# Samleo8/RadarSLAMPy

Measured on AMD Instinct MI355X. Metric: radar scan-pairs/sec (400x3768 polar), higher is better.
Workload: dtype u8/f32/f64

## Files before the change

profiles/time_doh.py:

```python
#!/usr/bin/env python3
import os, sys
sys.path.insert(0, os.path.dirname(os.path.dirname(os.path.abspath(__file__))))
import numpy as np
from radarslampy_amd import _ffi, synth
if os.environ.get("ROAM_LIB"):
    _ffi.LIB_PATH = os.path.abspath(os.environ["ROAM_LIB"])
from radarslampy_amd.engine import Engine
B = int(sys.argv[1]) if len(sys.argv) > 1 else 512
recs, poses, feat = synth.make_sequence(5, 2, n_static=460, n_movers=24, distortion=True)
ctx = _ffi.Context(0)
eng = Engine(B, 2 * B, ctx=ctx, retrack_on_device=True, retrack_slots=B)
for t in range(2):
    eng.upload_scan(t, recs[t])
for b in range(1, B):
    for t in range(2):
        eng.copy_scan(b * 2 + t, t)
eng.synchronize()
for b in range(B):
    eng.init_lane(b, b * 2, feat[:40], poses[0])
eng.step(np.arange(B, dtype=np.int32) * 2 + 1)
eng.synchronize()
for k in os.environ.get("KERNELS", "doh_integral,doh_det_maxima").split(","):
    ms, by = eng.time_kernel(k, 3)
    print(f"{k}: {ms:.2f} ms per {B} detections = {ms*1e3/B:.1f} us each, {by/ms/1e6:.0f} GB/s algorithmic")
eng.close(); ctx.close()
```

radarslampy_amd/csrc/retrack_det.hip:

```cpp
#include "doh_common.h"
#include "retrack_geom.h"

__device__ __forceinline__ void rt_push_maxima(const RtArgs &a, int ls, int r, int c, uint32_t bits, double v0, double v1)
{
#pragma unroll
    for (int l = 0; l < 2; l++)
        if ((bits >> l) & 1u) {
            const int o = atomicAdd(&a.cand_n[ls], 1);
            if (o < BP_MAX_PTS) {
                a.cand_rc[(int64_t)ls * BP_MAX_PTS + o] = ((uint32_t)r << 16) | ((uint32_t)c << 2) | (uint32_t)(l + 1);
                a.cand_val[(int64_t)ls * BP_MAX_PTS + o] = l ? v1 : v0;
            }
        }
}

#define SD_RING 64
#define SD_DUP 8
#define SD_PITCHB (SD_BP * 8)
#define SD_SPLIT 36
#define SD_THREADS (512 * SD_HALVES)
#define SD_RING_BYTES ((SD_RING + SD_DUP) * SD_PITCHB)
#define SD_M2_ROWS (SD_T + 2)
#define SD_LDS_BYTES (SD_RING_BYTES + 2 * SD_M2_ROWS * SD_PC * 8)
#define SD_NST ((SD_T * SD_BP + SD_THREADS - 1) / SD_THREADS)
extern __shared__ __align__(16) char sd_smem[];

#define SD_SCALE 0.0009765625
#define SD_UNSCALE 1024.0
__device__ __forceinline__ double sd_box(double a, double d, double b, double c)
{
    const double t = __dsub_rn(__dadd_rn(a, d), b);
    double r;
    asm("v_add_f64 %0, %1, -%2 clamp" : "=v"(r) : "v"(t), "v"(c));
    return r;
}
__device__ __forceinline__ double sd_max(double x, double y)
{
    double r;
    asm("v_max_f64 %0, %1, %2" : "=v"(r) : "v"(x), "v"(y));
    return r;
}
template <int SIZE> __device__ __forceinline__ double sd_wi() { return __dmul_rn(__ddiv_rn(__ddiv_rn(1.0, (double)SIZE), (double)SIZE), SD_UNSCALE); }

__device__ __forceinline__ double sd_ldr(const uint32_t (&ca)[12], const uint32_t (&cb)[12], int row, int j)
{
    const int rr = ((row % SD_RING) + SD_RING) % SD_RING;
    return rr < SD_SPLIT ? *reinterpret_cast<const double *>(sd_smem + (ca[j] + rr * SD_PITCHB))
                         : *reinterpret_cast<const double *>(sd_smem + (cb[j] + (rr - SD_SPLIT) * SD_PITCHB));
}

template <int PH>
__device__ __forceinline__ void sd_tile_fast(const uint32_t (&ca)[12], const uint32_t (&cb)[12], double (&d0)[SD_T / 8], double (&d1)[SD_T / 8])
{
    static_assert(SD_T == 16, "two positions per thread and step");
    double v[2][2][4];
    auto issue = [&](int i, double(&o)[2][4]) {
        const int L = (i >> 2) & 1, q = i & 3;
        const int SIZE = L ? 30 : 15, s2 = (SIZE - 1) / 2, s3 = SIZE / 3;
        const int ra = q < 2 ? -s3 + 1 : (q == 2 ? -s2 : -(s3 / 2)), rb = ra + (q < 2 ? 2 * s3 - 1 : (q == 2 ? SIZE : s3));
        const int ja = 6 * L + (q == 0 ? 0 : (q == 1 ? 2 : 4)), jb = ja + 1;
#pragma unroll
        for (int k = 0; k < 2; k++) {
            const int R0 = SD_T * PH + 8 * k;
            o[k][0] = sd_ldr(ca, cb, R0 + ra, ja); o[k][1] = sd_ldr(ca, cb, R0 + rb, jb);
            o[k][2] = sd_ldr(ca, cb, R0 + ra, jb); o[k][3] = sd_ldr(ca, cb, R0 + rb, ja);
        }
    };
    issue(0, v[0]);
    double mid[2] = {0.0, 0.0}, dxx[2] = {0.0, 0.0};
#pragma unroll
    for (int i = 0; i < 8; i++) {
        if (i + 1 < 8) issue(i + 1, v[(i + 1) & 1]);
        const int L = (i >> 2) & 1, q = i & 3;
        const double(&x)[2][4] = v[i & 1];
        double t0 = __dadd_rn(x[0][0], x[0][1]), t1 = __dadd_rn(x[1][0], x[1][1]);
        t0 = __dsub_rn(t0, x[0][2]); t1 = __dsub_rn(t1, x[1][2]);
        double b0, b1;
        asm("v_add_f64 %0, %1, -%2 clamp" : "=v"(b0) : "v"(t0), "v"(x[0][3]));
        asm("v_add_f64 %0, %1, -%2 clamp" : "=v"(b1) : "v"(t1), "v"(x[1][3]));
        if (q == 0 || q == 2) { mid[0] = b0; mid[1] = b1; }
        else {
            const double w_i = L ? sd_wi<30>() : sd_wi<15>();
            double m0 = __dmul_rn(3.0, b0), m1 = __dmul_rn(3.0, b1);
            double e0 = __dsub_rn(mid[0], m0), e1 = __dsub_rn(mid[1], m1);
            e0 = __dmul_rn(-e0, w_i); e1 = __dmul_rn(-e1, w_i);
            if (q == 1) { dxx[0] = e0; dxx[1] = e1; }
            else if (L) { d1[0] = __dmul_rn(dxx[0], e0); d1[1] = __dmul_rn(dxx[1], e1); }
            else { d0[0] = __dmul_rn(dxx[0], e0); d0[1] = __dmul_rn(dxx[1], e1); }
        }
        __builtin_amdgcn_sched_barrier(0);
    }
}

template <int SIZE, int L>
__device__ __forceinline__ double sd_det_rows(const uint32_t (&ca)[12], int w8, int r, int H)
{
    constexpr int s2 = (SIZE - 1) / 2, s3 = SIZE / 3, w = SIZE, J = 6 * L;
    const double w_i = sd_wi<SIZE>();
    auto ld = [&](int row, int j) { return *reinterpret_cast<const double *>(sd_smem + (ca[j] + (uint32_t)(((row & (SD_RING - 1)) - w8) * SD_PITCHB))); };
    const int xa = clipi(r - s3 + 1, 0, H - 1), xb = clipi(xa + 2 * s3 - 1, 0, H - 1);
    double mid = sd_box(ld(xa, J + 0), ld(xb, J + 1), ld(xa, J + 1), ld(xb, J + 0));
    double side = sd_box(ld(xa, J + 2), ld(xb, J + 3), ld(xa, J + 3), ld(xb, J + 2));
    double dxx = __dsub_rn(mid, __dmul_rn(3.0, side));
    dxx = __dmul_rn(-dxx, w_i);
    const int ya = clipi(r - s2, 0, H - 1), yb = clipi(ya + w, 0, H - 1), za = clipi(r - s3 / 2, 0, H - 1), zb = clipi(za + s3, 0, H - 1);
    mid = sd_box(ld(ya, J + 4), ld(yb, J + 5), ld(ya, J + 5), ld(yb, J + 4));
    side = sd_box(ld(za, J + 4), ld(zb, J + 5), ld(za, J + 5), ld(zb, J + 4));
    double dyy = __dsub_rn(mid, __dmul_rn(3.0, side));
    dyy = __dmul_rn(-dyy, w_i);
    return __dmul_rn(dxx, dyy);
}

template <int SIZE>
__device__ __forceinline__ double sd_dxy(double det, int r, int c, int H, int W, int cbase)
{
    constexpr int s3 = SIZE / 3;
    const double w_i = sd_wi<SIZE>();
    const int r0 = clipi(r - s3, 0, H - 1), r1 = clipi(r0 + s3, 0, H - 1), r2 = clipi(r + 1, 0, H - 1), r3 = clipi(r2 + s3, 0, H - 1);
    const int c0 = clipi(c - s3, 0, W - 1), c1 = clipi(c0 + s3, 0, W - 1), c2 = clipi(c + 1, 0, W - 1), c3 = clipi(c2 + s3, 0, W - 1);
    auto at = [&](int rr, int cc) { return *reinterpret_cast<const double *>(sd_smem + (((rr & (SD_RING - 1)) * SD_BP + (cc - cbase)) * 8)); };
    const double tl = sd_box(at(r0, c0), at(r1, c1), at(r0, c1), at(r1, c0));
    const double br = sd_box(at(r2, c2), at(r3, c3), at(r2, c3), at(r3, c2));
    const double bl = sd_box(at(r0, c2), at(r1, c3), at(r0, c3), at(r1, c2));
    const double tr = sd_box(at(r2, c0), at(r3, c1), at(r2, c1), at(r3, c0));
    double dxy = __dsub_rn(__dsub_rn(__dadd_rn(bl, tr), tl), br);
    dxy = __dmul_rn(-dxy, w_i);
    return __dsub_rn(det, __dmul_rn(0.81, __dmul_rn(dxy, dxy)));
}

__global__ __launch_bounds__(256) void rt_darktab_kernel(const uint32_t *__restrict__ map, int W, int cols, uint32_t *__restrict__ tab)
{
    const int H = W, strip = blockIdx.x, t = blockIdx.y, c0 = strip * SD_OUT;
    const int ra = max(SD_T * t - SD_HL, 0), rb = min(SD_T * t + SD_T - 1 + SD_HR, H - 1);
    const int xa = max(c0 - 1 - SD_HL, 0), xb = min(c0 - 1 + SD_PC - 1 + SD_HR, W - 1);
    const int nx = xb - xa + 1, n = max(0, rb - ra + 1) * max(0, nx);
    int lit = 0;
    for (int i = threadIdx.x; i < n; i += 256) {
        const int r = ra + i / nx, c = xa + i % nx;
        if ((int)(map[(int64_t)r * W + c] & 4095u) < cols) lit = 1;
    }
    lit = __syncthreads_or(lit);
    if (threadIdx.x == 0 && !lit) atomicOr(&tab[strip * SD_DT_WORDS + (t >> 5)], 1u << (t & 31));
}
__global__ __launch_bounds__(256) void rt_darkskip_kernel(int nt, uint32_t *__restrict__ tab)
{
    uint32_t *T = tab + blockIdx.x * SD_DT_WORDS;
    const int t = threadIdx.x;
    auto dark = [&](int q) { return q < 0 || q >= nt || ((T[q >> 5] >> (q & 31)) & 1u); };
    auto skip = [&](int j) { return dark(j - 1) && dark(j) && dark(j + 1); };
    if (skip(t + 4)) atomicOr(&T[8 + (t >> 5)], 1u << (t & 31));
    if (t == 0) {
        int first = nt, last = -1;
        for (int q = 0; q < nt; q++)
            if (!dark(q)) { if (first == nt) first = q; last = q; }
        T[16] = (uint32_t)first; T[17] = (uint32_t)last;
    }
}

template <int P> struct SdTag { static constexpr int value = P; };

__global__ __launch_bounds__(SD_THREADS) void rt_det_strip_kernel(RtArgs a, int first, int P, int nstrips)
{
    const int nact = min(P, max(0, *a.rt_n - first));
    if (a.fused && rt_one_sweep(a, first)) return;
    const int total = nact * nstrips, per = (total + 7) >> 3;
    const int xcd = blockIdx.x & 7, jq = blockIdx.x >> 3;
    const int work = xcd * per + jq;
    if (jq >= per || work >= total) return;
    const int ls = work / nstrips, strip = work - ls * nstrips;
    const int W = a.W, H = a.W, SP = a.SP;
    const double thr = a.threshold;
    typedef const uint32_t __attribute__((address_space(4))) *SdConstPtr;
    const SdConstPtr dtab = (SdConstPtr)(uintptr_t)(a.darktab + strip * SD_DT_WORDS);
    uint32_t dk_w = 0, skf_w = 0;
    const double *__restrict__ S = a.S + (int64_t)ls * SP * W;
    const int tid = threadIdx.x, lane = tid & 63;
    const int wave = __builtin_amdgcn_readfirstlane(tid >> 6), w8 = wave & 7, half = wave >> 3;
    const int c0 = strip * SD_OUT, cbase = c0 - 1 - SD_HL;
    const int pc = half * 64 + lane, c = c0 - 1 + pc;
    const bool cvalid = c >= 0 && c < W;
    const bool wave_live = c0 - 1 + half * 64 < W;
    constexpr int M2ROW = SD_PC * 8, M2BUF = SD_M2_ROWS * M2ROW;
    const uint32_t mb = (uint32_t)(SD_RING_BYTES + w8 * M2ROW + pc * 8);
    auto m2at = [&](int buf, int row, int dc) -> double & { return *reinterpret_cast<double *>(sd_smem + (mb + (uint32_t)(buf * M2BUF + (row - w8) * M2ROW + dc * 8))); };
    uint32_t ca[12], cb[12];
    {
        constexpr int off[6][2] = {{-7, 15}, {-2, 5}, {-4, 9}, {-14, 30}, {-5, 10}, {-9, 19}};
#pragma unroll
        for (int q = 0; q < 6; q++) {
            const int x0 = clipi(c + off[q][0], 0, W - 1), x1 = clipi(x0 + off[q][1], 0, W - 1);
            ca[2 * q] = (uint32_t)((w8 * SD_BP + (x0 - cbase)) * 8);
            ca[2 * q + 1] = (uint32_t)((w8 * SD_BP + (x1 - cbase)) * 8);
        }
#pragma unroll
        for (int q = 0; q < 12; q++) cb[q] = ca[q] + SD_SPLIT * SD_PITCHB;
    }
    const bool strip_inside = cbase >= 0 && cbase + SD_BP <= W;
    uint32_t goff[SD_NST], loff[SD_NST];
    int srow[SD_NST], scol[SD_NST];
#pragma unroll
    for (int j = 0; j < SD_NST; j++) {
        const int e = tid + SD_THREADS * j;
        srow[j] = e / SD_BP; scol[j] = e - srow[j] * SD_BP;
        goff[j] = (uint32_t)((srow[j] * SP + scol[j]) * 8);
        loff[j] = (uint32_t)(srow[j] * SD_PITCHB + scol[j] * 8);
    }
    double stage[2][SD_NST];
    const int nt = H / SD_T + 1;
    const int t_first = (int)dtab[16], t_last = (int)dtab[17];
    if (t_first >= nt) return;
    const int tb = t_first >= 1 ? ((t_first - 1) & ~3) : 0, te = min(nt, t_last + 2);
    int frow = SD_T * tb;
    auto fetch = [&](double(&st)[SD_NST], bool skip = false) {
        const bool whole = frow >= 0 && frow + SD_T <= H && strip_inside;
        const char *base = reinterpret_cast<const char *>(S + (int64_t)((skip && whole) ? 0 : frow) * SP + cbase);
        if (whole) {
#pragma unroll
            for (int j = 0; j < SD_NST; j++)
                if (SD_THREADS * (j + 1) <= SD_T * SD_BP || tid + SD_THREADS * j < SD_T * SD_BP) st[j] = *reinterpret_cast<const double *>(base + goff[j]);
        } else {
#pragma unroll
            for (int j = 0; j < SD_NST; j++) {
                const int gr = frow + srow[j], col = cbase + scol[j];
                if (srow[j] < SD_T && gr >= 0 && gr < H && col >= 0 && col < W) st[j] = *reinterpret_cast<const double *>(base + goff[j]);
            }
        }
        frow += SD_T;
    };
    auto put = [&](int quarter, const double(&st)[SD_NST]) {
#pragma unroll
        for (int j = 0; j < SD_NST; j++)
            if (SD_THREADS * (j + 1) <= SD_T * SD_BP || tid + SD_THREADS * j < SD_T * SD_BP) {
                double *d = reinterpret_cast<double *>(sd_smem + (loff[j] + (uint32_t)(quarter * SD_T * SD_PITCHB)));
                const double v = __dmul_rn(st[j], SD_SCALE);
                *d = v;
                if (quarter == 0 && srow[j] < SD_DUP) d[SD_RING * SD_BP] = v;
            }
    };
    double d0[SD_T / 8], d1[SD_T / 8], p0 = 0.0, p1 = 0.0;
    uint32_t cand = 0, pcand = 0;
#pragma unroll
    for (int k = 0; k < SD_T / 8; k++) { d0[k] = 0.0; d1[k] = 0.0; }
    auto decide = [&](int buf, int rr2, int r, double v0, double v1) {
        if (pc < 1 || pc > SD_OUT || c >= W || r >= H) return;
        double mx = m2at(buf, rr2, 0);
#pragma unroll
        for (int dr = -1; dr <= 1; dr++)
#pragma unroll
            for (int dc = -1; dc <= 1; dc++) { const double u = m2at(buf, rr2 + dr, dc); mx = u > mx ? u : mx; }
        const uint32_t bits = ((v0 > thr && !(mx > v0)) ? 1u : 0u) | ((v1 > thr && !(mx > v1)) ? 2u : 0u);
        if (bits) rt_push_maxima(a, first + ls, r, c, bits, v0, v1);
    };
    auto maxima = [&](int pt, int buf) {
        if (w8 == 7) {
            if (pcand) decide(buf, 1, SD_T * pt - 1, p0, p1);
            p0 = d0[SD_T / 8 - 1]; p1 = d1[SD_T / 8 - 1]; pcand = cand >> (SD_T / 8 - 1);
        }
        if (cand) {
#pragma unroll
            for (int k = 0; k < SD_T / 8; k++) {
                const int rr = 8 * k + w8;
                if (((cand >> k) & 1u) && rr < SD_T - 1) decide(buf, 2 + rr, SD_T * pt + rr, d0[k], d1[k]);
            }
        }
    };
    for (int i = tid; i < 2 * SD_M2_ROWS * SD_PC; i += SD_THREADS) reinterpret_cast<double *>(sd_smem + SD_RING_BYTES)[i] = 0.0;
    fetch(stage[1]);
    fetch(stage[0]);
    put(0, stage[1]);
    put(1, stage[0]);
    fetch(stage[1]);
    fetch(stage[0]);
    __syncthreads();
    auto step = [&](auto tag, int t) {
        constexpr int PH = decltype(tag)::value, WB = PH & 1;
        const uint32_t tb = 1u << (t & 31);
        put((PH + 2) & 3, stage[(PH + 1) & 1]);
        fetch(stage[(PH + 1) & 1], (skf_w & tb) != 0);
        if (t >= 1) maxima(t - 1, WB ^ 1);
        const int rbase = SD_T * t;
        const bool fast = t >= 1 && rbase + SD_T - 1 + SD_HR <= H - 1;
        const bool dark = (dk_w & tb) != 0;
        if (!wave_live || dark) {
#pragma unroll
            for (int k = 0; k < SD_T / 8; k++) { d0[k] = 0.0; d1[k] = 0.0; }
        } else if (fast) {
            sd_tile_fast<PH>(ca, cb, d0, d1);
        } else {
#pragma unroll
            for (int k = 0; k < SD_T / 8; k++) {
                const int r = rbase + 8 * k + w8;
                d0[k] = r < H ? sd_det_rows<15, 0>(ca, w8, r, H) : 0.0;
                d1[k] = r < H ? sd_det_rows<30, 1>(ca, w8, r, H) : 0.0;
            }
        }
        cand = 0;
#pragma unroll
        for (int k = 0; k < SD_T / 8; k++) {
            const int rr = 8 * k + w8, r = rbase + rr;
            double mx = sd_max(d0[k], d1[k]);
            if (mx > thr) {
                if (d0[k] > thr) d0[k] = sd_dxy<15>(d0[k], r, c, H, W, cbase);
                if (d1[k] > thr) d1[k] = sd_dxy<30>(d1[k], r, c, H, W, cbase);
                if (!cvalid) { d0[k] = 0.0; d1[k] = 0.0; }
                mx = sd_max(d0[k], d1[k]);
                if (mx > thr) cand |= 1u << k;
            }
            if (k == SD_T / 8 - 1 && w8 >= 6) m2at(WB, rr - (SD_T - 2), 0) = m2at(WB ^ 1, 2 + rr, 0);
            m2at(WB, 2 + rr, 0) = mx;
        }
        __syncthreads();
    };
    for (int t = tb; t < te; t += 4) {
        if ((t & 31) == 0 || t == tb) { dk_w = dtab[t >> 5]; skf_w = dtab[8 + (t >> 5)]; }
        step(SdTag<0>(), t);
        if (t + 1 < te) step(SdTag<1>(), t + 1);
        if (t + 2 < te) step(SdTag<2>(), t + 2);
        if (t + 3 < te) step(SdTag<3>(), t + 3);
    }
    maxima(te - 1, (te - 1) & 1);
}

#include "retrack_fused.inc"

size_t retrack_darktab_words(int W) { return (size_t)((W + SD_OUT - 1) / SD_OUT) * SD_DT_WORDS; }

hipError_t launch_retrack_darktab(hipStream_t st, const uint32_t *map, int W, int cols, uint32_t *darktab)
{
    const int ns = (W + SD_OUT - 1) / SD_OUT, nt = W / SD_T + 1;
    if (nt > 256) return hipErrorInvalidValue;
    hipLaunchKernelGGL(rt_darktab_kernel, dim3(ns, nt), dim3(256), 0, st, map, W, cols, darktab);
    hipLaunchKernelGGL(rt_darkskip_kernel, dim3(ns), dim3(256), 0, st, nt, darktab);
    return hipGetLastError();
}

size_t retrack_fused_boxtab_words(int W) { return 2 * (size_t)((W + SD_OUT - 1) / SD_OUT + 1) * (size_t)((W + SD_T - 1) / SD_T); }
size_t retrack_fused_halo_words(int W) { return (size_t)((W + SD_T - 1) / SD_T) * SD_T * FD_HALO; }

hipError_t launch_retrack_fused_tables(hipStream_t st, const uint32_t *map, int W, int cols, uint32_t *mapT, uint32_t *boxtab, uint32_t *darktab)
{
    const int nband = (W + SD_OUT - 1) / SD_OUT, nblk = (W + SD_T - 1) / SD_T;
    hipLaunchKernelGGL(rf_mapT_kernel, dim3((W + 31) / 32, (W + 31) / 32), dim3(256), 0, st, map, W, mapT);
    hipLaunchKernelGGL(rf_boxtab_kernel, dim3(nblk, nband + 1), dim3(64), 0, st, mapT, W, cols, nblk, boxtab);
    return launch_retrack_darktab(st, mapT, W, cols, darktab);
}

hipError_t retrack_det_init()
{
    if (hipError_t ef = hipFuncSetAttribute(reinterpret_cast<const void *>(rt_fused_kernel), hipFuncAttributeMaxDynamicSharedMemorySize, FD_LDS_BYTES); ef != hipSuccess) return ef;
    return hipFuncSetAttribute(reinterpret_cast<const void *>(rt_det_strip_kernel), hipFuncAttributeMaxDynamicSharedMemorySize, SD_LDS_BYTES);
}

hipError_t launch_det(hipStream_t st, const RtArgs &a, int first, int P)
{
    if (a.size1 != 15 || a.size2 != 30) return hipErrorInvalidValue;
    const int ns = (a.W + SD_OUT - 1) / SD_OUT;
    hipLaunchKernelGGL(rt_det_strip_kernel, dim3((unsigned)(((int64_t)P * ns + 7) / 8 * 8)), dim3(SD_THREADS), SD_LDS_BYTES, st, a, first, P, ns);
    return hipGetLastError();
}

hipError_t launch_retrack_fused(hipStream_t st, const RtArgs &a, int first, int P, int dbg)
{
    hipLaunchKernelGGL(rt_fused_kernel, dim3(P), dim3(FD_THREADS), FD_LDS_BYTES, st, a, first, dbg);
    return hipGetLastError();
}
```

Measured before the change: 57930.

## Skip dxx side-box evaluation in DoH fast tile when bound cannot exceed threshold

The fast DoH tile path now evaluates the dyy terms and the dxx middle box first. It then computes a conservative upper bound on the Hessian determinant per wave, using a small relative and absolute slack, and loads and evaluates the dxx side box only when some lane could pass the threshold. This cuts LDS reads and f64 arithmetic for dark or low-response tiles. The cost is an extra ballot and bound computation plus branch divergence across waves, and exactness depends on the bound being truly conservative. A profiling script that measures the screen pass rate is also added.

```diff
diff --git a/profiles/det_screen_rate.py b/profiles/det_screen_rate.py
--- /dev/null
+++ b/profiles/det_screen_rate.py
@@ -0,0 +1,54 @@
+#!/usr/bin/env python3
+import os
+import sys
+
+ROOT = os.path.dirname(os.path.dirname(os.path.abspath(__file__)))
+sys.path.insert(0, ROOT)
+sys.path.insert(0, os.path.join(ROOT, "tests"))
+import numpy as np
+
+import oracle
+import det_candidate_cases as dc
+import det_screen_model as m
+
+THR = dc.THRESHOLD
+
+
+def scans(which):
+    from radarslampy_amd import synth
+    if which == "real":
+        pay = np.load(os.path.join(ROOT, "tests", "golden", "tiny_track.npz"))["payload"]
+        for t in (0, len(pay) // 2, len(pay) - 1):
+            yield "real scan %d (tests/golden/tiny_track.npz)" % t, pay[t].astype(np.float32) / np.float32(255.)
+        return
+    if which == "bench":
+        import bench
+        work = bench.WORK_RETRACK
+    else:
+        work = dict(n_static=460, n_movers=24)
+    recs = synth.make_sequence(5, 2, distortion=True, **work)[0]
+    yield "%s workload, seed 5 frame 1 %s" % (which, work), oracle.extractDataFromRadarImage(recs[1])[0]
+
+
+def table(name, polar):
+    cart = oracle.convertPolarImageToCartesian(polar)
+    S = dc.integral(cart)
+    lit = ~dc.dark_steps(polar.shape[1], polar.shape[0])
+    print("%s: image %d x %d, %.1f %% of the strip-steps lit" % (name, cart.shape[0], cart.shape[1], 100.0 * lit.mean()))
+    print("  %-28s %21s   %21s" % ("quantity (size 15 / size 30)", "positions", "waves"))
+    rows = {"dxy needed": [], "dyy -> xx-side not ruled out": [], "dxx -> yy-side not ruled out": []}
+    for size in m.SIZES:
+        for key, exact in (("dyy -> xx-side not ruled out", "dyy"), ("dxx -> yy-side not ruled out", "dxx")):
+            need, passing, fast = m.waves(S, size, THR, exact)
+            sel = lit[:, :, None] & fast[None, :, None] & np.ones(8, bool)
+            assert not (passing & ~need).any(), "a passing product was ruled out"
+            rows[key].append((need[sel].mean(), need.any(axis=-1)[sel].mean()))
+        rows["dxy needed"].append((passing[sel].mean(), passing.any(axis=-1)[sel].mean()))
+    for key, ((p15, w15), (p30, w30)) in rows.items():
+        print("  %-28s %8.2f %% / %6.2f %%   %8.1f %% / %6.1f %%" % (key, 100 * p15, 100 * p30, 100 * w15, 100 * w30))
+
+
+if __name__ == "__main__":
+    for which in (sys.argv[1:] or ["bench", "steady", "real"]):
+        for name, polar in scans(which):
+            table(name, polar)
diff --git a/profiles/time_doh.py b/profiles/time_doh.py
--- a/profiles/time_doh.py
+++ b/profiles/time_doh.py
@@ -7,7 +7,14 @@
     _ffi.LIB_PATH = os.path.abspath(os.environ["ROAM_LIB"])
 from radarslampy_amd.engine import Engine
 B = int(sys.argv[1]) if len(sys.argv) > 1 else 512
-recs, poses, feat = synth.make_sequence(5, 2, n_static=460, n_movers=24, distortion=True)
+WORKLOAD = sys.argv[2] if len(sys.argv) > 2 else "steady"
+if WORKLOAD == "bench":
+    import bench
+    WORK = bench.WORK_RETRACK
+else:
+    assert WORKLOAD == "steady", WORKLOAD
+    WORK = dict(n_static=460, n_movers=24)
+recs, poses, feat = synth.make_sequence(5, 2, distortion=True, **WORK)
 ctx = _ffi.Context(0)
 eng = Engine(B, 2 * B, ctx=ctx, retrack_on_device=True, retrack_slots=B)
 for t in range(2):
@@ -22,5 +29,5 @@
 eng.synchronize()
 for k in os.environ.get("KERNELS", "doh_integral,doh_det_maxima").split(","):
     ms, by = eng.time_kernel(k, 3)
-    print(f"{k}: {ms:.2f} ms per {B} detections = {ms*1e3/B:.1f} us each, {by/ms/1e6:.0f} GB/s algorithmic")
+    print(f"{WORKLOAD} {k}: {ms:.2f} ms per {B} detections = {ms*1e3/B:.1f} us each, {by/ms/1e6:.0f} GB/s algorithmic")
 eng.close(); ctx.close()
diff --git a/radarslampy_amd/csrc/retrack_det.hip b/radarslampy_amd/csrc/retrack_det.hip
--- a/radarslampy_amd/csrc/retrack_det.hip
+++ b/radarslampy_amd/csrc/retrack_det.hip
@@ -49,13 +49,14 @@
                          : *reinterpret_cast<const double *>(sd_smem + (cb[j] + (rr - SD_SPLIT) * SD_PITCHB));
 }
 
+#define SD_SKIP_REL 9.5367431640625e-07
+#define SD_SKIP_ABS 3.814697265625e-06
 template <int PH>
-__device__ __forceinline__ void sd_tile_fast(const uint32_t (&ca)[12], const uint32_t (&cb)[12], double (&d0)[SD_T / 8], double (&d1)[SD_T / 8])
+__device__ __forceinline__ void sd_tile_fast(const uint32_t (&ca)[12], const uint32_t (&cb)[12], double thr_s, double (&d0)[SD_T / 8], double (&d1)[SD_T / 8])
 {
     static_assert(SD_T == 16, "two positions per thread and step");
     double v[2][2][4];
-    auto issue = [&](int i, double(&o)[2][4]) {
-        const int L = (i >> 2) & 1, q = i & 3;
+    auto issue = [&](int L, int q, double(&o)[2][4]) {
         const int SIZE = L ? 30 : 15, s2 = (SIZE - 1) / 2, s3 = SIZE / 3;
         const int ra = q < 2 ? -s3 + 1 : (q == 2 ? -s2 : -(s3 / 2)), rb = ra + (q < 2 ? 2 * s3 - 1 : (q == 2 ? SIZE : s3));
         const int ja = 6 * L + (q == 0 ? 0 : (q == 1 ? 2 : 4)), jb = ja + 1;
@@ -66,29 +67,47 @@
             o[k][2] = sd_ldr(ca, cb, R0 + ra, jb); o[k][3] = sd_ldr(ca, cb, R0 + rb, ja);
         }
     };
-    issue(0, v[0]);
-    double mid[2] = {0.0, 0.0}, dxx[2] = {0.0, 0.0};
-#pragma unroll
-    for (int i = 0; i < 8; i++) {
-        if (i + 1 < 8) issue(i + 1, v[(i + 1) & 1]);
-        const int L = (i >> 2) & 1, q = i & 3;
-        const double(&x)[2][4] = v[i & 1];
+    auto boxes = [&](const double(&x)[2][4], double(&b)[2]) {
         double t0 = __dadd_rn(x[0][0], x[0][1]), t1 = __dadd_rn(x[1][0], x[1][1]);
         t0 = __dsub_rn(t0, x[0][2]); t1 = __dsub_rn(t1, x[1][2]);
-        double b0, b1;
-        asm("v_add_f64 %0, %1, -%2 clamp" : "=v"(b0) : "v"(t0), "v"(x[0][3]));
-        asm("v_add_f64 %0, %1, -%2 clamp" : "=v"(b1) : "v"(t1), "v"(x[1][3]));
-        if (q == 0 || q == 2) { mid[0] = b0; mid[1] = b1; }
-        else {
-            const double w_i = L ? sd_wi<30>() : sd_wi<15>();
-            double m0 = __dmul_rn(3.0, b0), m1 = __dmul_rn(3.0, b1);
-            double e0 = __dsub_rn(mid[0], m0), e1 = __dsub_rn(mid[1], m1);
-            e0 = __dmul_rn(-e0, w_i); e1 = __dmul_rn(-e1, w_i);
-            if (q == 1) { dxx[0] = e0; dxx[1] = e1; }
-            else if (L) { d1[0] = __dmul_rn(dxx[0], e0); d1[1] = __dmul_rn(dxx[1], e1); }
-            else { d0[0] = __dmul_rn(dxx[0], e0); d0[1] = __dmul_rn(dxx[1], e1); }
+        asm("v_add_f64 %0, %1, -%2 clamp" : "=v"(b[0]) : "v"(t0), "v"(x[0][3]));
+        asm("v_add_f64 %0, %1, -%2 clamp" : "=v"(b[1]) : "v"(t1), "v"(x[1][3]));
+    };
+    auto deriv = [&](int L, const double(&mid)[2], const double(&side)[2], double(&e)[2]) {
+        const double w_i = L ? sd_wi<30>() : sd_wi<15>();
+        const double m0 = __dmul_rn(3.0, side[0]), m1 = __dmul_rn(3.0, side[1]);
+        const double e0 = __dsub_rn(mid[0], m0), e1 = __dsub_rn(mid[1], m1);
+        e[0] = __dmul_rn(-e0, w_i); e[1] = __dmul_rn(-e1, w_i);
+    };
+    issue(0, 2, v[0]);
+    double mid[2], b[2], dyy[2][2], xm[2][2];
+    bool need[2];
+#pragma unroll
+    for (int i = 0; i < 6; i++) {
+        const int L = i / 3, j = i % 3;
+        if (i + 1 < 6) issue((i + 1) / 3, (i + 1) % 3 == 0 ? 2 : ((i + 1) % 3 == 1 ? 3 : 0), v[(i + 1) & 1]);
+        boxes(v[i & 1], j == 0 ? mid : (j == 1 ? b : xm[L]));
+        if (j == 1) deriv(L, mid, b, dyy[L]);
+        if (j == 2) {
+            const double w1 = __dmul_rn(L ? sd_wi<30>() : sd_wi<15>(), 1.0 + SD_SKIP_REL), w2 = __dmul_rn(2.0, w1);
+            const double u0 = __dmul_rn(__dmul_rn(fabs(dyy[L][0]), xm[L][0]), dyy[L][0] > 0.0 ? w2 : w1);
+            const double u1 = __dmul_rn(__dmul_rn(fabs(dyy[L][1]), xm[L][1]), dyy[L][1] > 0.0 ? w2 : w1);
+            need[L] = __builtin_amdgcn_ballot_w64(u0 > thr_s || u1 > thr_s) != 0;
         }
         __builtin_amdgcn_sched_barrier(0);
+    }
+    if (need[0]) issue(0, 1, v[0]);
+    if (need[1]) issue(1, 1, v[1]);
+    d0[0] = 0.0; d0[1] = 0.0; d1[0] = 0.0; d1[1] = 0.0;
+    if (need[0]) {
+        double e[2];
+        boxes(v[0], b); deriv(0, xm[0], b, e);
+        d0[0] = __dmul_rn(e[0], dyy[0][0]); d0[1] = __dmul_rn(e[1], dyy[0][1]);
+    }
+    if (need[1]) {
+        double e[2];
+        boxes(v[1], b); deriv(1, xm[1], b, e);
+        d1[0] = __dmul_rn(e[0], dyy[1][0]); d1[1] = __dmul_rn(e[1], dyy[1][1]);
     }
 }
 
@@ -169,7 +188,7 @@
     if (jq >= per || work >= total) return;
     const int ls = work / nstrips, strip = work - ls * nstrips;
     const int W = a.W, H = a.W, SP = a.SP;
-    const double thr = a.threshold;
+    const double thr = a.threshold, thr_s = __dsub_rn(thr, SD_SKIP_ABS);
     typedef const uint32_t __attribute__((address_space(4))) *SdConstPtr;
     const SdConstPtr dtab = (SdConstPtr)(uintptr_t)(a.darktab + strip * SD_DT_WORDS);
     uint32_t dk_w = 0, skf_w = 0;
@@ -285,7 +304,7 @@
 #pragma unroll
             for (int k = 0; k < SD_T / 8; k++) { d0[k] = 0.0; d1[k] = 0.0; }
         } else if (fast) {
-            sd_tile_fast<PH>(ca, cb, d0, d1);
+            sd_tile_fast<PH>(ca, cb, thr_s, d0, d1);
         } else {
 #pragma unroll
             for (int k = 0; k < SD_T / 8; k++) {
```

Measured after the change: 58770 (median of 6 runs). 1.01x the previous value.
